# alazarteka/Self-Forcing

Hardware: AMD Instinct MI355X
Metric: decoded frames/sec/node, Wan-1.3B 832x480 4-step AR rollout (higher is better)
Workload: dtype bf16

## Files before the change

self-forcing_amd/csrc/dit_forward.hip:

```cpp
#include <algorithm>
#include "sf_host.h"

int sf_internal_write_kv_indices(void* buf, int layers, int64_t global_end, int64_t local_end, void* stream);

namespace {

struct Work {
  void *x, *xn, *qkv, *q, *att, *hbuf, *cols, *headout, *sin, *etmp, *e, *e0, *ctx1, *ctx;
  void* xq;
  float* xs;
  size_t total;
};

constexpr int FP8_MAX_SEGMENTS = 8;

Work carve(const sf_model* m, void* ws, int B, int F, int lat_h, int lat_w, int groups) {
  const size_t M = (size_t)B * F * (lat_h / 2) * (lat_w / 2);
  const size_t C = m->dim, BG = (size_t)B * groups, T = (size_t)B * m->text_len;
  Carve c(ws);
  Work w;
  w.x = c.take(M * C * 2);
  w.xn = c.take(M * C * 2);
  w.qkv = c.take(M * 3 * C * 2);
  w.q = c.take(M * C * 2);
  w.att = c.take(M * C * 2);
  w.hbuf = c.take(M * (size_t)m->ffn_dim * 2);
  w.cols = c.take(M * (size_t)m->in_dim * 4 * 2);
  w.headout = c.take(M * (size_t)m->out_dim * 4 * 2);
  w.sin = c.take(BG * m->freq_dim * 2);
  w.etmp = c.take(BG * C * 2);
  w.e = c.take(BG * C * 2);
  w.e0 = c.take(BG * 6 * C * 2);
  w.ctx1 = c.take(T * C * 2);
// ... 157 lines not shown
    const int T = B * m->text_len;
    SF_TRY(lin(Gemm(a->prompt_embeds, m->text_dim, m->text0_w, m->text_dim, ws.ctx1, C, T, C, m->text_dim).bias(m->text0_b).epi(SF_EPI_BIAS_GELU)
                   .fp8w(m->text0_q, m->text0_s, T)));
    SF_TRY(lin(Gemm(ws.ctx1, C, m->text2_w, C, ws.ctx, C, T, C, C).bias(m->text2_b).fp8w(m->text2_q, m->text2_s, T)));
    if (f8) SF_TRY(sf_quantize_fp8(ws.ctx, C, T, C, T, ws.xq, ws.xs, stream));
    for (int l = 0; l < m->num_layers; ++l) {
      const sf_layer_weights& lw = m->layers_host[l];
      const sf_layer_fp8& lq = f8 ? m->layers_fp8_host[l] : no_fp8;
      SF_TRY(run(Gemm(ws.ctx, C, lw.ckv_w, C, a->ck_cache_host[l], C, T, C, C).bias(lw.ckv_b).fp8w(lq.ckv_q, lq.ckv_s, T)));
      SF_TRY(sf_rmsnorm(a->ck_cache_host[l], C, lw.cnorm_k_w, a->ck_cache_host[l], C, T, C, m->eps, stream));
      SF_TRY(run(Gemm(ws.ctx, C, bptr(lw.ckv_w, (size_t)C * C), C, a->cv_cache_host[l], C, T, C, C).bias(bptr(lw.ckv_b, C))
                     .fp8w(f8 ? (const char*)lq.ckv_q + (size_t)C * C : nullptr, f8 ? lq.ckv_s + C : nullptr, T)));
    }
    if (cross_keys) SF_TRY(sf_cross_fold_scan(a->ck_cache_host, a->cv_cache_host, m->num_layers, B, m->text_len, C, cross_keys, cross_log2w, stream));
    if (im) {
      const ImgWork iw = carve_img(m, im, a->workspace, ws.total, B);
      const int R = B * im->clip_len, D = im->clip_dim;
      void* ctx_raw = iw.ctx;
      void* ctx_img = (void*)bptr(iw.ctx, (size_t)R * C);
      SF_TRY(sf_layernorm_rows(ia->clip_feature, im->img_ln0_w, im->img_ln0_b, iw.t0, R, D, im->img_eps, stream));
      SF_TRY(Gemm(iw.t0, D, im->img_fc1_w, D, iw.t1, D, R, D, D).bias(im->img_fc1_b).bf16(stream));
      SF_TRY(sf_clip_gelu(iw.t1, iw.t1, (int64_t)R * D, stream));
      SF_TRY(Gemm(iw.t1, D, im->img_fc2_w, D, ctx_raw, C, R, C, D).bias(im->img_fc2_b).bf16(stream));
      SF_TRY(sf_layernorm_affine(ctx_raw, im->img_ln1_w, im->img_ln1_b, ctx_img, R, C, im->img_eps, stream));
      for (int l = 0; l < m->num_layers; ++l) {
        const sf_i2v_layer& il = im->layers_host[l];
        SF_TRY(Gemm(ctx_img, C, il.kvimg_w, C, ia->kimg_cache_host[l], C, R, C, C).bias(il.kvimg_b).bf16(stream));
        SF_TRY(sf_rmsnorm(ia->kimg_cache_host[l], C, il.norm_k_img_w, ia->kimg_cache_host[l], C, R, C, m->eps, stream));
        SF_TRY(Gemm(ctx_img, C, bptr(il.kvimg_w, (size_t)C * C), C, ia->vimg_cache_host[l], C, R, C, C).bias(bptr(il.kvimg_b, C)).bf16(stream));
      }
    }
  }

  for (int l = 0; l < m->num_layers; ++l) {
    const sf_layer_weights& lw = m->layers_host[l];
    const sf_layer_fp8& lq = f8 ? m->layers_fp8_host[l] : no_fp8;
    const void* mod = lw.modulation;
    const bool last_layer = l == m->num_layers - 1;
    SF_TRY(sf_layernorm_modulate(ws.x, ws.xn, Mt, C, m->eps, bptr(mod, 0), bptr(mod, C), bptr(ws.e0, 0), bptr(ws.e0, C), 6L * C, rpg, stream));
    SF_TRY(lin(Gemm(ws.xn, C, lw.qkv_w, C, ws.qkv, 3 * C, Mt, 3 * C, C).bias(lw.qkv_b).fp8w(lq.qkv_q, lq.qkv_s, M)));
    for (int p = 0; p < np; ++p) {
      const sf_forward_args* q = ps[p];
      const size_t roff = (size_t)p * M;
      if (q->evict > 0) {
        SF_TRY(sf_kv_evict(q->k_cache_host[l], B, q->cache_tokens, C, q->sink_tokens, q->evict, q->keep, q->evict_scratch, q->evict_scratch_bytes, stream));
        SF_TRY(sf_kv_evict(q->v_cache_host[l], B, q->cache_tokens, C, q->sink_tokens, q->evict, q->keep, q->evict_scratch, q->evict_scratch_bytes, stream));
      }
      SF_TRY(sf_qkv_norm_rope_cache(bptr(ws.qkv, roff * 3 * C), lw.norm_q_w, lw.norm_k_w, (void*)bptr(ws.q, roff * C), q->k_cache_host[l], q->v_cache_host[l],
                                    m->rope_cos, m->rope_sin, B, F, h, w, C, m->num_heads, q->cache_tokens, q->write_start, q->start_frame, m->eps, stream));
      if (q->cache_only && last_layer) continue;
      SF_TRY(Attention(bptr(ws.q, roff * C), C, (long)L * C, bptr(q->k_cache_host[l], (size_t)q->attn_start * C), bptr(q->v_cache_host[l], (size_t)q->attn_start * C),
                       C, cache_b, (void*)bptr(ws.att, roff * C), C, (long)L * C, B, m->num_heads, L, q->attn_end - q->attn_start).run(stream));
    }
    const int p0 = last_layer ? first_full : 0;
    if (p0 == np) return finish_indices();
    const size_t r0 = (size_t)p0 * M;
    const int Mr = (np - p0) * M;
    void* x = (void*)bptr(ws.x, r0 * C);
    void* xn = (void*)bptr(ws.xn, r0 * C);
    void* qb = (void*)bptr(ws.q, r0 * C);
    void* att = (void*)bptr(ws.att, r0 * C);
    void* hb = (void*)bptr(ws.hbuf, r0 * m->ffn_dim);
    const void* e0r = bptr(ws.e0, (size_t)p0 * BG * 6 * C);
    SF_TRY(lin(Gemm(att, C, lw.o_w, C, x, C, Mr, C, C).bias(lw.o_b).epi(SF_EPI_BIAS_GATE_RESID).resid(x, C)
                   .gate(bptr(mod, 2 * (size_t)C), bptr(e0r, 2 * (size_t)C), 6L * C, rpg).fp8w(lq.o_q, lq.o_s, M)));
    SF_TRY(sf_layernorm_affine(x, lw.norm3_w, lw.norm3_b, xn, Mr, C, m->eps, stream));
    SF_TRY(lin(Gemm(xn, C, lw.cq_w, C, qb, C, Mr, C, C).bias(lw.cq_b).fp8w(lq.cq_q, lq.cq_s, M)));
    SF_TRY(sf_rmsnorm(qb, C, lw.cnorm_q_w, qb, C, Mr, C, m->eps, stream));
    for (int p = p0; p < np; ++p)
      SF_TRY(Attention(bptr(ws.q, (size_t)p * M * C), C, (long)L * C, a->ck_cache_host[l], a->cv_cache_host[l], C, ctx_b, (void*)bptr(ws.att, (size_t)p * M * C), C,
                       (long)L * C, B, m->num_heads, L, m->text_len)
                 .fold(cross_keys ? cross_keys + (size_t)l * B : nullptr, cross_keys ? cross_log2w + (size_t)l * B : nullptr).run(stream));
    if (im)
      SF_TRY(Attention(ws.q, C, (long)L * C, ia->kimg_cache_host[l], ia->vimg_cache_host[l], C, (long)im->clip_len * C, ws.att, C, (long)L * C, B, m->num_heads, L,
                       im->clip_len).accum().run(stream));
    SF_TRY(lin(Gemm(att, C, lw.co_w, C, x, C, Mr, C, C).bias(lw.co_b).epi(SF_EPI_BIAS_RESID).resid(x, C).fp8w(lq.co_q, lq.co_s, M)));
    SF_TRY(sf_layernorm_modulate(x, xn, Mr, C, m->eps, bptr(mod, 3 * (size_t)C), bptr(mod, 4 * (size_t)C), bptr(e0r, 3 * (size_t)C),
                                 bptr(e0r, 4 * (size_t)C), 6L * C, rpg, stream));
    SF_TRY(lin(Gemm(xn, C, lw.ffn0_w, C, hb, m->ffn_dim, Mr, m->ffn_dim, C).bias(lw.ffn0_b).epi(SF_EPI_BIAS_GELU).fp8w(lq.ffn0_q, lq.ffn0_s, M)));
    SF_TRY(lin(Gemm(hb, m->ffn_dim, lw.ffn2_w, m->ffn_dim, x, C, Mr, C, m->ffn_dim).bias(lw.ffn2_b).epi(SF_EPI_BIAS_GATE_RESID).resid(x, C)
                   .gate(bptr(mod, 5 * (size_t)C), bptr(e0r, 5 * (size_t)C), 6L * C, rpg).fp8w(lq.ffn2_q, lq.ffn2_s, M)));
  }
// ... 15 lines not shown
```

self-forcing_amd/csrc/elementwise.hip:

```cpp
#include "sf_common.h"
#include "../../include/sf_hip.h"

namespace {

constexpr int ROWS_PER_BLOCK = 4;

template <int NCH>
__device__ __forceinline__ void load_row(const bf16_t* row, int lane, float (&v)[NCH][8]) {
#pragma unroll
  for (int i = 0; i < NCH; ++i) {
    const bf16x8 t = *reinterpret_cast<const bf16x8*>(row + (i * 64 + lane) * 8);
#pragma unroll
    for (int j = 0; j < 8; ++j) v[i][j] = (float)t[j];
  }
}

template <int NCH>
__device__ __forceinline__ void ln_stats(const float (&v)[NCH][8], int C, float eps, float& mean, float& rstd) {
  float s = 0.f;
#pragma unroll
  for (int i = 0; i < NCH; ++i)
#pragma unroll
    for (int j = 0; j < 8; ++j) s += v[i][j];
  mean = wave_sum(s) / (float)C;
// ... 70 lines not shown
#pragma unroll
      for (int j = 0; j < 8; ++j)
        o[j] = (bf16_t)((v[i][j] - mean) * rstd * (MODE == 0 ? 1.0f + (float)scl[i][j] : (float)scl[i][j]) + (float)add[i][j]);
      *reinterpret_cast<bf16x8*>(out + (long)row * C + (i * 64 + lane) * 8) = o;
    }
  }
}

template <int NCH>
__global__ __launch_bounds__(256) void rmsnorm_kernel(const bf16_t* __restrict__ x, int ldx, const bf16_t* __restrict__ w,
                                                      bf16_t* __restrict__ out, int ldo, int M, int C, float eps) {
  const int lane = threadIdx.x & 63;
  const int row = blockIdx.x * ROWS_PER_BLOCK + (threadIdx.x >> 6);
  if (row >= M) return;
  float v[NCH][8];
  load_row<NCH>(x + (long)row * ldx, lane, v);
  float q = 0.f;
#pragma unroll
  for (int i = 0; i < NCH; ++i)
#pragma unroll
    for (int j = 0; j < 8; ++j) q += v[i][j] * v[i][j];
  const float r = rsqrtf(wave_sum(q) / (float)C + eps);
#pragma unroll
  for (int i = 0; i < NCH; ++i) {
    const int e = (i * 64 + lane) * 8;
    const bf16x8 wt = *reinterpret_cast<const bf16x8*>(w + e);
    bf16x8 o;
#pragma unroll
    for (int j = 0; j < 8; ++j) o[j] = (bf16_t)((float)(bf16_t)(v[i][j] * r) * (float)wt[j]);
    *reinterpret_cast<bf16x8*>(out + (long)row * ldo + e) = o;
  }
}

template <int NCH>
__global__ __launch_bounds__(256) void qkv_norm_rope_cache_kernel(
    const bf16_t* __restrict__ qkv, const bf16_t* __restrict__ wq, const bf16_t* __restrict__ wk,
    bf16_t* __restrict__ q_out, bf16_t* __restrict__ k_cache, bf16_t* __restrict__ v_cache,
    const float* __restrict__ rope_cos, const float* __restrict__ rope_sin, int rows, int L, int hgt, int wid, int C,
    long cache_tokens, int write_start, int start_frame, float eps, int c0, int c1) {
  const int lane = threadIdx.x & 63;
  const int row = blockIdx.x * ROWS_PER_BLOCK + (threadIdx.x >> 6);
  if (row >= rows) return;
  const int b = row / L, t = row - b * L;
  const int fi = t / (hgt * wid), rem = t - fi * (hgt * wid);
  const int hi = rem / wid, wi = rem - hi * wid;
  const int pos_t = start_frame + fi;
  const bf16_t* src = qkv + (long)row * 3 * C;
  const long crow = ((long)b * cache_tokens + write_start + t) * C;

#pragma unroll
  for (int i = 0; i < NCH; ++i) {
    const int e = (i * 64 + lane) * 8;
    *reinterpret_cast<u32x4*>(v_cache + crow + e) = *reinterpret_cast<const u32x4*>(src + 2 * C + e);
  }

#pragma unroll
  for (int which = 0; which < 2; ++which) {
    float v[NCH][8];
    load_row<NCH>(src + which * C, lane, v);
    float q = 0.f;
#pragma unroll
    for (int i = 0; i < NCH; ++i)
#pragma unroll
      for (int j = 0; j < 8; ++j) q += v[i][j] * v[i][j];
    const float r = rsqrtf(wave_sum(q) / (float)C + eps);
    const bf16_t* wn = which ? wk : wq;
    bf16_t* dst = which ? (k_cache + crow) : (q_out + (long)row * C);
#pragma unroll
    for (int i = 0; i < NCH; ++i) {
      const int e = (i * 64 + lane) * 8;
      const bf16x8 wt = *reinterpret_cast<const bf16x8*>(wn + e);
      const int pair0 = (e & 127) >> 1;
      bf16x8 o;
#pragma unroll
      for (int pp = 0; pp < 4; ++pp) {
        const int pj = pair0 + pp;
        const int pos = pj < c0 ? pos_t : (pj < c0 + c1 ? hi : wi);
        const float cs = rope_cos[pos * 64 + pj];
        const float sn = rope_sin[pos * 64 + pj];
        const float re = (float)(bf16_t)((float)(bf16_t)(v[i][2 * pp] * r) * (float)wt[2 * pp]);
        const float im = (float)(bf16_t)((float)(bf16_t)(v[i][2 * pp + 1] * r) * (float)wt[2 * pp + 1]);
        o[2 * pp] = (bf16_t)(re * cs - im * sn);
        o[2 * pp + 1] = (bf16_t)(re * sn + im * cs);
      }
      *reinterpret_cast<bf16x8*>(dst + e) = o;
    }
  }
}

__global__ __launch_bounds__(256) void copy_rows_kernel(const char* __restrict__ src, long src_bstride,
                                                        char* __restrict__ dst, long dst_bstride, long bytes_per_batch) {
  const long n16 = bytes_per_batch >> 4;
  const char* s = src + (long)blockIdx.y * src_bstride;
  char* d = dst + (long)blockIdx.y * dst_bstride;
  for (long i = (long)blockIdx.x * blockDim.x + threadIdx.x; i < n16; i += (long)gridDim.x * blockDim.x)
    reinterpret_cast<u32x4*>(d)[i] = reinterpret_cast<const u32x4*>(s)[i];
}

__global__ __launch_bounds__(256) void patchify_kernel(const bf16_t* __restrict__ x, bf16_t* __restrict__ cols, long total,
                                                       int Cin, int H, int W) {
  const int h2 = H >> 1, w2 = W >> 1;
  for (long i = (long)blockIdx.x * blockDim.x + threadIdx.x; i < total; i += (long)gridDim.x * blockDim.x) {
    const int cch = (int)(i % Cin);
    long r = i / Cin;
    const int ww = (int)(r % w2); r /= w2;
    const int hh = (int)(r % h2);
    const long bf = r / h2;
    const bf16_t* s = x + ((bf * Cin + cch) * H + 2 * hh) * (long)W + 2 * ww;
    bf16x4 o;
    o[0] = s[0]; o[1] = s[1]; o[2] = s[W]; o[3] = s[W + 1];
    *reinterpret_cast<bf16x4*>(cols + ((bf * h2 + hh) * w2 + ww) * (long)(Cin * 4) + cch * 4) = o;
  }
}

__device__ __forceinline__ double block_sigma_lookup(double t, const float* __restrict__ sigmas,
                                                     const float* __restrict__ timesteps, int n_table) {
// ... 144 lines not shown
                                     const void* mod_scale, const void* e0_shift, const void* e0_scale,
                                     int64_t e0_group_stride, int rows_per_group, void* stream) {
  SF_CHECK(x && out && mod_shift && mod_scale && e0_shift && e0_scale, "sf_layernorm_modulate: null tensor");
  SF_CHECK(M > 0 && channels_ok(C), "sf_layernorm_modulate: unsupported shape M=%d C=%d (C must be 512*{1,2,3,4,5,6,8,10})", M, C);
  SF_CHECK(rows_per_group > 0 && e0_group_stride % 8 == 0, "sf_layernorm_modulate: bad group layout");
  return launch_layernorm<0>((const bf16_t*)x, (bf16_t*)out, M, C, eps, (const bf16_t*)mod_shift, (const bf16_t*)mod_scale,
                             (const bf16_t*)e0_shift, (const bf16_t*)e0_scale, e0_group_stride, rows_per_group,
                             "sf_layernorm_modulate", (hipStream_t)stream);
}

extern "C" int sf_layernorm_affine(const void* x, const void* weight, const void* bias, void* out, int M, int C,
                                   float eps, void* stream) {
  SF_CHECK(x && out && weight && bias, "sf_layernorm_affine: null tensor");
  SF_CHECK(M > 0 && channels_ok(C), "sf_layernorm_affine: unsupported shape M=%d C=%d", M, C);
  return launch_layernorm<1>((const bf16_t*)x, (bf16_t*)out, M, C, eps, (const bf16_t*)weight, (const bf16_t*)bias, nullptr,
                             nullptr, 0, 1, "sf_layernorm_affine", (hipStream_t)stream);
}

extern "C" int sf_rmsnorm(const void* x, int ldx, const void* weight, void* out, int ldo, int M, int C, float eps,
                          void* stream) {
  SF_CHECK(x && out && weight, "sf_rmsnorm: null tensor");
  SF_CHECK(M > 0 && channels_ok(C) && ldx >= C && ldo >= C && ldx % 8 == 0 && ldo % 8 == 0, "sf_rmsnorm: unsupported shape M=%d C=%d", M, C);
  const dim3 grid((M + ROWS_PER_BLOCK - 1) / ROWS_PER_BLOCK), block(256);
  hipStream_t s = (hipStream_t)stream;
  switch (C / 512) {
#define SF_RMS_CASE(N) \
  case N: return sf_launch<&rmsnorm_kernel<N>>("sf_rmsnorm", grid, block, 0, s, (const bf16_t*)x, ldx, (const bf16_t*)weight, (bf16_t*)out, ldo, M, C, eps);
    SF_RMS_CASE(1) SF_RMS_CASE(2) SF_RMS_CASE(3) SF_RMS_CASE(4) SF_RMS_CASE(5) SF_RMS_CASE(6) SF_RMS_CASE(8) SF_RMS_CASE(10)
#undef SF_RMS_CASE
    default: SF_CHECK(false, "sf_rmsnorm: unsupported channel count %d", C);
  }
}

extern "C" int sf_qkv_norm_rope_cache(const void* qkv, const void* norm_q_w, const void* norm_k_w, void* q_out,
                                      void* k_cache, void* v_cache, const float* rope_cos, const float* rope_sin,
                                      int B, int f, int h, int w, int C, int num_heads, int64_t cache_tokens,
                                      int write_start, int start_frame, float eps, void* stream) {
  SF_CHECK(qkv && norm_q_w && norm_k_w && q_out && k_cache && v_cache && rope_cos && rope_sin, "sf_qkv_norm_rope_cache: null tensor");
  SF_CHECK(B > 0 && f > 0 && h > 0 && w > 0 && channels_ok(C), "sf_qkv_norm_rope_cache: unsupported shape");
  SF_CHECK(num_heads > 0 && C == num_heads * 128, "sf_qkv_norm_rope_cache: head_dim must be 128 (C=%d heads=%d)", C, num_heads);
  const int L = f * h * w;
  SF_CHECK(write_start >= 0 && (int64_t)write_start + L <= cache_tokens, "sf_qkv_norm_rope_cache: cache overflow: write_start=%d + L=%d > capacity=%lld",
           write_start, L, (long long)cache_tokens);
  SF_CHECK(start_frame >= 0 && start_frame + f <= 1024 && h <= 1024 && w <= 1024, "sf_qkv_norm_rope_cache: RoPE position out of the 1024-entry table");
  const int rows = B * L;
  const dim3 grid((rows + ROWS_PER_BLOCK - 1) / ROWS_PER_BLOCK), block(256);
  hipStream_t s = (hipStream_t)stream;
  const int c = 64, c1 = c / 3, c0 = c - 2 * c1;
  switch (C / 512) {
#define SF_QKV_CASE(N)                                                                                                                         \
  case N: return sf_launch<&qkv_norm_rope_cache_kernel<N>>("sf_qkv_norm_rope_cache", grid, block, 0, s, (const bf16_t*)qkv, (const bf16_t*)norm_q_w, \
                             (const bf16_t*)norm_k_w, (bf16_t*)q_out, (bf16_t*)k_cache, (bf16_t*)v_cache, rope_cos, rope_sin,                    \
                             rows, L, h, w, C, (long)cache_tokens, write_start, start_frame, eps, c0, c1);
    SF_QKV_CASE(1) SF_QKV_CASE(2) SF_QKV_CASE(3) SF_QKV_CASE(4) SF_QKV_CASE(5) SF_QKV_CASE(6) SF_QKV_CASE(8) SF_QKV_CASE(10)
#undef SF_QKV_CASE
    default: SF_CHECK(false, "sf_qkv_norm_rope_cache: unsupported channel count %d", C);
  }
}

extern "C" int sf_kv_evict(void* cache, int B, int64_t cache_tokens, int row_elems, int sink, int evict, int keep,
                           void* scratch, size_t scratch_bytes, void* stream) {
  SF_CHECK(cache && B > 0 && row_elems > 0 && (row_elems % 8) == 0, "sf_kv_evict: bad arguments");
  SF_CHECK(sink >= 0 && evict >= 0 && keep >= 0 && (int64_t)sink + evict + keep <= cache_tokens, "sf_kv_evict: window out of range");
  if (evict == 0 || keep == 0) return 0;
  const long row_b = (long)row_elems * 2;
  const long bytes = (long)keep * row_b;
  SF_CHECK(scratch && scratch_bytes >= (size_t)(bytes * B), "sf_kv_evict: scratch too small (%zu < %ld)", scratch_bytes, bytes * B);
  char* base = (char*)cache;
  const long bstride = (long)cache_tokens * row_b;
  const int gx = (int)min((long)2048, (bytes / 16 + 255) / 256);
  const dim3 grid(gx, B), block(256);
  hipStream_t s = (hipStream_t)stream;
  SF_TRY(sf_launch<&copy_rows_kernel>("sf_kv_evict", grid, block, 0, s, base + (long)(sink + evict) * row_b, bstride, (char*)scratch, bytes, bytes));
  return sf_launch<&copy_rows_kernel>("sf_kv_evict", grid, block, 0, s, (const char*)scratch, bytes, base + (long)sink * row_b, bstride, bytes);
}

extern "C" int sf_patchify(const void* x, void* cols, int B, int F, int Cin, int H, int W, void* stream) {
  SF_CHECK(x && cols && B > 0 && F > 0 && Cin > 0, "sf_patchify: bad arguments");
  SF_CHECK(H % 2 == 0 && W % 2 == 0, "sf_patchify: latent H=%d W=%d must be even (patch 2x2)", H, W);
  const long total = (long)B * F * (H / 2) * (W / 2) * Cin;
  const int gx = (int)min((long)4096, (total + 255) / 256);
  return sf_launch<&patchify_kernel>("sf_patchify", dim3(gx), dim3(256), 0, (hipStream_t)stream, (const bf16_t*)x, (bf16_t*)cols, total, Cin, H, W);
}

extern "C" int sf_unpatchify_x0(const void* head_out, const void* xt, const void* timestep, int t_is_int64,
                                const float* sigmas, const float* timesteps, int n_table, void* flow, void* x0,
                                int B, int F, int groups, int Cout, int H, int W, void* stream) {
  SF_CHECK(head_out && xt && timestep && sigmas && timesteps && flow && x0, "sf_unpatchify_x0: null tensor");
  SF_CHECK(B > 0 && F > 0 && groups > 0 && F % groups == 0, "sf_unpatchify_x0: frames=%d not divisible by groups=%d", F, groups);
  SF_CHECK(H % 2 == 0 && W % 2 == 0 && n_table > 0, "sf_unpatchify_x0: bad shape");
// ... 104 lines not shown
```

self-forcing_amd/csrc/gemm_bf16.hip:

```cpp
#include <type_traits>
#include "sf_common.h"
#include "lds_dma.h"
#include "../../include/sf_hip.h"

namespace {

constexpr int BM = 128, BN = 128, BK = 64;
constexpr int GEMM_THREADS = 256;
constexpr int TILE_BYTES = BM * BK * 2;
constexpr int STAGE_BYTES = 2 * TILE_BYTES;
constexpr int GEMM_LDS = 2 * STAGE_BYTES;

struct GemmP {
  const bf16_t* a;
  const bf16_t* w;
  const bf16_t* bias;
  bf16_t* out;
  const bf16_t* resid;
  const bf16_t* gate_mod;
  const bf16_t* gate_e0;
  long gate_group_stride;
  int rows_per_group;
  int M, N, K, lda, ldw, ldo, ldr;
  int tiles_m, tiles_n;
  long a_bs, w_bs, o_bs, r_bs;
  const float* a_scale;
  const float* w_scale;
  int rows_per_seg;
};

typedef int i32x4 __attribute__((ext_vector_type(4)));
typedef int i32x8 __attribute__((ext_vector_type(8)));

__device__ __forceinline__ f32x4 mfma_f8(const bf16x8& w0, const bf16x8& w1, const bf16x8& x0, const bf16x8& x1, const f32x4& acc) {
  const i32x8 wv = __builtin_shufflevector(__builtin_bit_cast(i32x4, w0), __builtin_bit_cast(i32x4, w1), 0, 1, 2, 3, 4, 5, 6, 7);
  const i32x8 xv = __builtin_shufflevector(__builtin_bit_cast(i32x4, x0), __builtin_bit_cast(i32x4, x1), 0, 1, 2, 3, 4, 5, 6, 7);
  return __builtin_amdgcn_mfma_scale_f32_16x16x128_f8f6f4(wv, xv, acc, 0, 0, 0, 127, 0, 127);
}

template <int MT>
__device__ __forceinline__ void fp8_scale_acc(const GemmP& p, f32x4 (&acc)[MT][4], int m_base, int n_base, int lane) {
  f32x4 ws[4];
#pragma unroll
  for (int nt = 0; nt < 4; ++nt) ws[nt] = *reinterpret_cast<const f32x4*>(p.w_scale + min(n_base + nt * 16 + (lane >> 4) * 4, p.N - 4));
#pragma unroll
  for (int mt = 0; mt < MT; ++mt) {
    const float sa = p.a_scale[min(m_base + mt * 16 + (lane & 15), p.M - 1) / p.rows_per_seg];
#pragma unroll
    for (int nt = 0; nt < 4; ++nt)
#pragma unroll
      for (int j = 0; j < 4; ++j) acc[mt][nt][j] = acc[mt][nt][j] * (sa * ws[nt][j]);
  }
}

template <int EPI>
__device__ __forceinline__ bf16x4 epi_apply(const GemmP& p, const f32x4& a4, int m, int n, const bf16_t* e0row) {
  float y[4];
#pragma unroll
  for (int j = 0; j < 4; ++j) y[j] = a4[j];
  if (p.bias) {
    const bf16x4 b = *reinterpret_cast<const bf16x4*>(p.bias + n);
#pragma unroll
    for (int j = 0; j < 4; ++j) y[j] += (float)b[j];
  }
  if (EPI == SF_EPI_BIAS_GELU) {
#pragma unroll
    for (int j = 0; j < 4; ++j) y[j] = gelu_tanh_f(y[j]);
  }
  if (EPI == SF_EPI_BIAS_GATE_RESID) {
    const bf16x4 gm = *reinterpret_cast<const bf16x4*>(p.gate_mod + n);
    const bf16x4 ge = *reinterpret_cast<const bf16x4*>(e0row + n);
#pragma unroll
    for (int j = 0; j < 4; ++j) y[j] *= (float)(bf16_t)((float)gm[j] + (float)ge[j]);
  }
  if (EPI == SF_EPI_BIAS_RESID || EPI == SF_EPI_BIAS_GATE_RESID) {
    const bf16x4 rv = *reinterpret_cast<const bf16x4*>(p.resid + (long)m * p.ldr + n);
#pragma unroll
    for (int j = 0; j < 4; ++j) y[j] += (float)rv[j];
  }
  bf16x4 o;
#pragma unroll
  for (int j = 0; j < 4; ++j) o[j] = (bf16_t)y[j];
  return o;
}

template <int EPI, int MT>
__device__ __forceinline__ void gemm_epilogue(const GemmP& p, f32x4 (&acc)[MT][4], int mrow, int ncol) {
#pragma unroll
  for (int mt = 0; mt < MT; ++mt) {
    const int m = mrow + mt * 16;
    if (m >= p.M) continue;
    const bf16_t* e0row = nullptr;
    if (EPI == SF_EPI_BIAS_GATE_RESID) e0row = p.gate_e0 + (long)(m / p.rows_per_group) * p.gate_group_stride;
#pragma unroll
    for (int nt = 0; nt < 4; ++nt) {
      const int n = ncol + nt * 16;
      if (n >= p.N) continue;
      if (EPI == SF_EPI_F32) {
        *reinterpret_cast<f32x4*>(reinterpret_cast<float*>(p.out) + (long)m * p.ldo + n) = acc[mt][nt];
        continue;
      }
      *reinterpret_cast<bf16x4*>(p.out + (long)m * p.ldo + n) = epi_apply<EPI>(p, acc[mt][nt], m, n, e0row);
    }
  }
}

template <int EPI>
__device__ __forceinline__ bf16x4 epi_math(const f32x4& a4, const bf16x4& b, const bf16x4& gm, const bf16x4& ge, const bf16x4& rv) {
  float y[4];
#pragma unroll
  for (int j = 0; j < 4; ++j) y[j] = a4[j] + (float)b[j];
  if (EPI == SF_EPI_BIAS_GELU) {
#pragma unroll
    for (int j = 0; j < 4; ++j) y[j] = gelu_tanh_f(y[j]);
  }
  if (EPI == SF_EPI_BIAS_GATE_RESID) {
#pragma unroll
    for (int j = 0; j < 4; ++j) y[j] *= (float)(bf16_t)((float)gm[j] + (float)ge[j]);
  }
  if (EPI == SF_EPI_BIAS_RESID || EPI == SF_EPI_BIAS_GATE_RESID) {
#pragma unroll
    for (int j = 0; j < 4; ++j) y[j] += (float)rv[j];
  }
  bf16x4 o;
#pragma unroll
  for (int j = 0; j < 4; ++j) o[j] = (bf16_t)y[j];
  return o;
}

template <int EPI, int MT>
__device__ __forceinline__ void gemm_epilogue_lds(const GemmP& p, f32x4 (&acc)[MT][4], int m_base, int n_base, char* wbuf, int lane) {
  const int r16 = lane & 15, cg = lane >> 4;
  constexpr bool GATE = EPI == SF_EPI_BIAS_GATE_RESID;
  constexpr bool RESID = EPI == SF_EPI_BIAS_RESID || EPI == SF_EPI_BIAS_GATE_RESID;
  const bf16x4 zero4 = {(bf16_t)0.f, (bf16_t)0.f, (bf16_t)0.f, (bf16_t)0.f};
// ... 13 lines not shown
#pragma unroll
    for (int nt = 0; nt < 4; ++nt) gm_v[nt] = *reinterpret_cast<const bf16x4*>(p.gate_mod + ncol[nt]);
  }
  constexpr int MB = 4;
#pragma unroll
  for (int m0 = 0; m0 < MT; m0 += MB) {
    bf16x4 rv[MB][4], ge[MB][4];
#pragma unroll
    for (int i = 0; i < MB; ++i) {
      if (m0 + i >= MT) break;
      const int m = min(m_base + (m0 + i) * 16 + r16, p.M - 1);
      const bf16_t* e0row = GATE ? p.gate_e0 + (long)(m / p.rows_per_group) * p.gate_group_stride : nullptr;
#pragma unroll
      for (int nt = 0; nt < 4; ++nt) {
        rv[i][nt] = RESID ? *reinterpret_cast<const bf16x4*>(p.resid + (long)m * p.ldr + ncol[nt]) : zero4;
        ge[i][nt] = GATE ? *reinterpret_cast<const bf16x4*>(e0row + ncol[nt]) : zero4;
      }
    }
#pragma unroll
    for (int i = 0; i < MB; ++i) {
      if (m0 + i >= MT) break;
      const int row = (m0 + i) * 16 + r16;
#pragma unroll
      for (int nt = 0; nt < 4; ++nt) {
        const int col = nt * 16 + cg * 4;
        const bf16x4 o = epi_math<EPI>(acc[m0 + i][nt], bias_v[nt], gm_v[nt], ge[i][nt], rv[i][nt]);
        const int chunk = (col >> 3) ^ (row & 7);
        *reinterpret_cast<bf16x4*>(wbuf + row * 128 + (chunk << 4) + (col & 4) * 2) = o;
      }
    }
  }
  __builtin_amdgcn_s_waitcnt(0xc07f);
  const int rr = lane >> 3, ch = lane & 7;
#pragma unroll
  for (int i = 0; i < 2 * MT; ++i) {
    const int row = i * 8 + rr;
    const int m = m_base + row, n = n_base + ch * 8;
    const bf16x8 v = *reinterpret_cast<const bf16x8*>(wbuf + row * 128 + ((ch ^ (row & 7)) << 4));
    if (m < p.M && n < p.N) *reinterpret_cast<bf16x8*>(p.out + (long)m * p.ldo + n) = v;
  }
}

template <int EPI, bool F8>
__global__ __launch_bounds__(GEMM_THREADS, 2) void gemm_bf16_kernel(GemmP p) {
  extern __shared__ __attribute__((aligned(16))) char smem[];
  const int tid = threadIdx.x;
  const int lane = tid & 63;
  const int wave = __builtin_amdgcn_readfirstlane(tid >> 6);

  if (blockIdx.y) {
    const long bz = blockIdx.y;
    p.a += bz * p.a_bs; p.w += bz * p.w_bs;
    if (EPI == SF_EPI_F32) p.out = reinterpret_cast<bf16_t*>(reinterpret_cast<float*>(p.out) + bz * p.o_bs); else p.out += bz * p.o_bs;
    if (p.resid) p.resid += bz * p.r_bs;
  }
  const int nwg = gridDim.x, bid = blockIdx.x;
  const int wg = sf_xcd_remap(bid, nwg);
  constexpr int GROUP_M = 8;
  const int width = GROUP_M * p.tiles_n;
  const int group = wg / width, first_m = group * GROUP_M;
  const int gsz = min(p.tiles_m - first_m, GROUP_M);
  const int in_group = wg - group * width;
  const int tm = first_m + in_group % gsz, tn = in_group / gsz;
  const int m0 = tm * BM, n0 = tn * BN;

  const bf16_t* a_src[4];
// ... 494 lines not shown
    return st == SF_GEMM_PP256 ? launch_pp_epi<8, F8>(p, a->epilogue, name, s)
         : st == SF_GEMM_PP224 ? launch_pp_epi<7, F8>(p, a->epilogue, name, s)
         : st == SF_GEMM_PP192 ? launch_pp_epi<6, F8>(p, a->epilogue, name, s) : launch_pp2_epi<F8>(p, a->epilogue, name, s);
  const int batch = a->batch > 1 ? a->batch : 1;
  p.a_bs = a->a_bstride; p.w_bs = a->w_bstride; p.o_bs = a->o_bstride; p.r_bs = a->r_bstride;
  SF_CHECK(batch == 1 || (a->a_bstride % 8 == 0 && a->w_bstride % 8 == 0 && a->o_bstride % 4 == 0 && a->r_bstride % 4 == 0),
           "%s: batch strides must keep 16-byte (operands) / 8-byte (output) alignment", name);
  const dim3 grid(p.tiles_m * p.tiles_n, batch), block(GEMM_THREADS);
  switch (a->epilogue) {
    case SF_EPI_BIAS: return sf_launch<&gemm_bf16_kernel<SF_EPI_BIAS, F8>>(name, grid, block, GEMM_LDS, s, p);
    case SF_EPI_BIAS_GELU: return sf_launch<&gemm_bf16_kernel<SF_EPI_BIAS_GELU, F8>>(name, grid, block, GEMM_LDS, s, p);
    case SF_EPI_BIAS_RESID: return sf_launch<&gemm_bf16_kernel<SF_EPI_BIAS_RESID, F8>>(name, grid, block, GEMM_LDS, s, p);
    case SF_EPI_BIAS_GATE_RESID: return sf_launch<&gemm_bf16_kernel<SF_EPI_BIAS_GATE_RESID, F8>>(name, grid, block, GEMM_LDS, s, p);
    case SF_EPI_F32:
      if constexpr (F8) {
        SF_CHECK(false, "%s: the raw fp32 epilogue is bf16-only", name);
      } else {
        SF_CHECK((uintptr_t)a->out % 16 == 0, "%s: fp32 output must be 16-byte aligned", name);
        return sf_launch<&gemm_bf16_kernel<SF_EPI_F32, false>>(name, grid, block, GEMM_LDS, s, p);
      }
    default: SF_CHECK(false, "%s: unknown epilogue %d", name, a->epilogue);
  }
}

void fill_params(const sf_gemm_args* a, GemmP& p, int unit) {
  p.a = (const bf16_t*)a->a; p.w = (const bf16_t*)a->w; p.bias = (const bf16_t*)a->bias;
  p.out = (bf16_t*)a->out; p.resid = (const bf16_t*)a->resid;
  p.gate_mod = (const bf16_t*)a->gate_mod; p.gate_e0 = (const bf16_t*)a->gate_e0;
  p.gate_group_stride = a->gate_group_stride; p.rows_per_group = a->rows_per_group;
  p.M = a->M; p.N = a->N; p.K = a->K / unit; p.lda = a->lda / unit; p.ldw = a->ldw / unit; p.ldo = a->ldo; p.ldr = a->ldr;
  p.tiles_n = (a->N + BN - 1) / BN;
  p.tiles_m = (a->M + BM - 1) / BM;
  p.a_scale = nullptr; p.w_scale = nullptr; p.rows_per_seg = 1;
}

}

extern "C" int sf_gemm_bf16(const sf_gemm_args* a, void* stream) {
  if (const int rc = check_args(a, "sf_gemm_bf16", BK)) return rc;
  GemmP p;
  fill_params(a, p, 1);
  return run_gemm<false>(a, p, "sf_gemm_bf16", (hipStream_t)stream);
}

extern "C" int sf_gemm_fp8(const sf_gemm_args* a, const float* a_scale, int rows_per_segment, const float* w_scale, void* stream) {
  if (const int rc = check_args(a, "sf_gemm_fp8", 2 * BK)) return rc;
  SF_CHECK(a->batch <= 1, "sf_gemm_fp8: batched products are bf16-only");
  SF_CHECK(a_scale && w_scale && rows_per_segment > 0, "sf_gemm_fp8: needs a_scale, w_scale and rows_per_segment > 0");
  SF_CHECK((uintptr_t)w_scale % 16 == 0, "sf_gemm_fp8: w_scale must be 16-byte aligned");
  GemmP p;
  fill_params(a, p, 2);
  p.a_scale = a_scale; p.w_scale = w_scale; p.rows_per_seg = rows_per_segment;
  return run_gemm<true>(a, p, "sf_gemm_fp8", (hipStream_t)stream);
}
```

self-forcing_amd/csrc/sf_host.h:

```cpp
#pragma once
#include <cstring>
#include "sf_common.h"
#include "../../include/sf_hip.h"

inline int sf_hip_ok(hipError_t e, const char* who, const char* what) {
  SF_CHECK(e == hipSuccess, "%s: %s failed: %s", who, what, hipGetErrorString(e));
  return 0;
}

struct Carve {
  char* base;
  size_t off;
  explicit Carve(void* p) : base((char*)p), off(0) {}
  char* take(size_t bytes) {
    char* r = base ? base + off : nullptr;
    off += (bytes + 255) & ~(size_t)255;
    return r;
  }
};

struct Gemm {
  sf_gemm_args g;
  const void* wq = nullptr;
  const float* w_scale = nullptr;
  int rows_per_segment = 0;
  Gemm(const void* a, int lda, const void* w, int ldw, void* out, int ldo, int M, int N, int K) {
    memset(&g, 0, sizeof(g));
    g.a = a; g.lda = lda; g.w = w; g.ldw = ldw; g.out = out; g.ldo = ldo; g.M = M; g.N = N; g.K = K;
    g.epilogue = SF_EPI_BIAS;
    g.rows_per_group = 1;
  }
  Gemm& bias(const void* b) { g.bias = b; return *this; }
  Gemm& epi(int e) { g.epilogue = e; return *this; }
  Gemm& resid(const void* r, int ldr) { g.resid = r; g.ldr = ldr; return *this; }
  Gemm& gate(const void* gate_mod, const void* gate_e0, long group_stride, int rows_per_group) {
    g.gate_mod = gate_mod; g.gate_e0 = gate_e0; g.gate_group_stride = group_stride; g.rows_per_group = rows_per_group;
    return *this;
  }
  Gemm& batch(int n, long a_bstride, long w_bstride, long o_bstride) {
    g.batch = n; g.a_bstride = a_bstride; g.w_bstride = w_bstride; g.o_bstride = o_bstride;
    return *this;
  }
  Gemm& fp8w(const void* w_e4m3, const float* scale, int rows_per_seg) {
    wq = w_e4m3; w_scale = scale; rows_per_segment = rows_per_seg;
    return *this;
  }
  int bf16(void* stream) const { return sf_gemm_bf16(&g, stream); }
  int fp8(const void* aq, const float* a_scale, void* stream) const {
    sf_gemm_args q = g;
    q.a = aq; q.lda = g.K; q.w = wq;
    return sf_gemm_fp8(&q, a_scale, rows_per_segment, w_scale, stream);
  }
};

struct Attention {
  sf_attention_args a;
  Attention(const void* q, long q_stride, long q_bstride, const void* k, const void* v, long kv_stride, long kv_bstride, void* out,
            long o_stride, long o_bstride, int B, int H, int Lq, int Lk) {
    memset(&a, 0, sizeof(a));
    a.q = q; a.q_stride = q_stride; a.q_bstride = q_bstride;
    a.k = k; a.v = v; a.kv_stride = kv_stride; a.kv_bstride = kv_bstride;
    a.out = out; a.o_stride = o_stride; a.o_bstride = o_bstride;
    a.B = B; a.H = H; a.Lq = Lq; a.Lk = Lk;
    a.structure = SF_ATTN_AUTO;
  }
  Attention& structure(int s) { a.structure = s; return *this; }
  Attention& accum() { a.accumulate = 1; return *this; }
  Attention& fold(const int32_t* keys, const float* log2w) { a.keys = keys; a.log2w = log2w; return *this; }
  int run(void* stream) const { return sf_attention(&a, stream); }
};
```

Baseline: 95.73.

## Write V columns of QKV GEMM directly into the KV cache

Adds a split-store epilogue to the bf16/fp8 GEMM so output columns past 2*C (the V projection) go straight into the per-layer V cache at each pass's write_start. The separate V copy in the qkv norm/rope kernel is then skipped. The kernel also preloads Q/K rows and rope tables up front. This removes one read and write of the V slice per layer. It is on by default but falls back when eviction is active or the two passes' cache regions overlap, and it adds per-row address math in the GEMM epilogue.

```diff
diff --git a/self-forcing_amd/csrc/dit_forward.hip b/self-forcing_amd/csrc/dit_forward.hip
--- a/self-forcing_amd/csrc/dit_forward.hip
+++ b/self-forcing_amd/csrc/dit_forward.hip
@@ -1,4 +1,5 @@
 #include <algorithm>
+#include <cstdlib>
 #include "sf_host.h"
 
 int sf_internal_write_kv_indices(void* buf, int layers, int64_t global_end, int64_t local_end, void* stream);
@@ -222,13 +223,32 @@
     }
   }
 
+  bool v_direct = true;
+  if (const char* e = getenv("SF_V_DIRECT")) v_direct = !(e[0] == '0' && e[1] == 0);
+  for (int p = 0; p < np; ++p) v_direct = v_direct && ps[p]->evict <= 0;
+  if (np == 2) {
+    const sf_forward_args *p0 = ps[0], *p1 = ps[1];
+    const int w1 = p1->write_start;
+    v_direct = v_direct && (w1 + L <= p0->attn_start || w1 >= p0->attn_end) && (w1 + L <= p0->write_start || w1 >= p0->write_start + L);
+  }
+  int qkv_structure = SF_GEMM_AUTO;
+  if (const char* e = getenv("SF_V_DIRECT_GEMM")) qkv_structure = atoi(e);
+
   for (int l = 0; l < m->num_layers; ++l) {
     const sf_layer_weights& lw = m->layers_host[l];
     const sf_layer_fp8& lq = f8 ? m->layers_fp8_host[l] : no_fp8;
     const void* mod = lw.modulation;
     const bool last_layer = l == m->num_layers - 1;
     SF_TRY(sf_layernorm_modulate(ws.x, ws.xn, Mt, C, m->eps, bptr(mod, 0), bptr(mod, C), bptr(ws.e0, 0), bptr(ws.e0, C), 6L * C, rpg, stream));
-    SF_TRY(lin(Gemm(ws.xn, C, lw.qkv_w, C, ws.qkv, 3 * C, Mt, 3 * C, C).bias(lw.qkv_b).fp8w(lq.qkv_q, lq.qkv_s, M)));
+    sf_gemm_split vsplit = {};
+    if (v_direct) {
+      vsplit.dst = a->v_cache_host[l];
+      vsplit.split_n = 2 * C; vsplit.ld = C;
+      vsplit.rows_per_sample = L; vsplit.samples = B; vsplit.passes = np;
+      vsplit.sample_rows = (long)a->cache_tokens; vsplit.sample_stride = cache_b;
+      for (int p = 0; p < np; ++p) vsplit.first_row[p] = ps[p]->write_start;
+    }
+    SF_TRY(lin(Gemm(ws.xn, C, lw.qkv_w, C, ws.qkv, 3 * C, Mt, 3 * C, C).bias(lw.qkv_b).fp8w(lq.qkv_q, lq.qkv_s, M).structure(qkv_structure).split(vsplit)));
     for (int p = 0; p < np; ++p) {
       const sf_forward_args* q = ps[p];
       const size_t roff = (size_t)p * M;
@@ -236,8 +256,12 @@
         SF_TRY(sf_kv_evict(q->k_cache_host[l], B, q->cache_tokens, C, q->sink_tokens, q->evict, q->keep, q->evict_scratch, q->evict_scratch_bytes, stream));
         SF_TRY(sf_kv_evict(q->v_cache_host[l], B, q->cache_tokens, C, q->sink_tokens, q->evict, q->keep, q->evict_scratch, q->evict_scratch_bytes, stream));
       }
-      SF_TRY(sf_qkv_norm_rope_cache(bptr(ws.qkv, roff * 3 * C), lw.norm_q_w, lw.norm_k_w, (void*)bptr(ws.q, roff * C), q->k_cache_host[l], q->v_cache_host[l],
-                                    m->rope_cos, m->rope_sin, B, F, h, w, C, m->num_heads, q->cache_tokens, q->write_start, q->start_frame, m->eps, stream));
+      if (v_direct)
+        SF_TRY(sf_internal_qk_norm_rope_cache(bptr(ws.qkv, roff * 3 * C), lw.norm_q_w, lw.norm_k_w, (void*)bptr(ws.q, roff * C), q->k_cache_host[l], m->rope_cos,
+                                              m->rope_sin, B, F, h, w, C, m->num_heads, q->cache_tokens, q->write_start, q->start_frame, m->eps, stream));
+      else
+        SF_TRY(sf_qkv_norm_rope_cache(bptr(ws.qkv, roff * 3 * C), lw.norm_q_w, lw.norm_k_w, (void*)bptr(ws.q, roff * C), q->k_cache_host[l], q->v_cache_host[l],
+                                      m->rope_cos, m->rope_sin, B, F, h, w, C, m->num_heads, q->cache_tokens, q->write_start, q->start_frame, m->eps, stream));
       if (q->cache_only && last_layer) continue;
       SF_TRY(Attention(bptr(ws.q, roff * C), C, (long)L * C, bptr(q->k_cache_host[l], (size_t)q->attn_start * C), bptr(q->v_cache_host[l], (size_t)q->attn_start * C),
                        C, cache_b, (void*)bptr(ws.att, roff * C), C, (long)L * C, B, m->num_heads, L, q->attn_end - q->attn_start).run(stream));
diff --git a/self-forcing_amd/csrc/elementwise.hip b/self-forcing_amd/csrc/elementwise.hip
--- a/self-forcing_amd/csrc/elementwise.hip
+++ b/self-forcing_amd/csrc/elementwise.hip
@@ -126,7 +126,7 @@
   }
 }
 
-template <int NCH>
+template <int NCH, bool COPY_V>
 __global__ __launch_bounds__(256) void qkv_norm_rope_cache_kernel(
     const bf16_t* __restrict__ qkv, const bf16_t* __restrict__ wq, const bf16_t* __restrict__ wk,
     bf16_t* __restrict__ q_out, bf16_t* __restrict__ k_cache, bf16_t* __restrict__ v_cache,
@@ -142,16 +142,40 @@
   const bf16_t* src = qkv + (long)row * 3 * C;
   const long crow = ((long)b * cache_tokens + write_start + t) * C;
 
+  bf16x8 raw[2][NCH];
+#pragma unroll
+  for (int which = 0; which < 2; ++which)
+#pragma unroll
+    for (int i = 0; i < NCH; ++i) raw[which][i] = *reinterpret_cast<const bf16x8*>(src + which * C + (i * 64 + lane) * 8);
+  float cs[NCH][4], sn[NCH][4];
 #pragma unroll
   for (int i = 0; i < NCH; ++i) {
-    const int e = (i * 64 + lane) * 8;
-    *reinterpret_cast<u32x4*>(v_cache + crow + e) = *reinterpret_cast<const u32x4*>(src + 2 * C + e);
+    const int pair0 = (((i * 64 + lane) * 8) & 127) >> 1;
+#pragma unroll
+    for (int pp = 0; pp < 4; ++pp) {
+      const int pj = pair0 + pp;
+      const int pos = pj < c0 ? pos_t : (pj < c0 + c1 ? hi : wi);
+      cs[i][pp] = rope_cos[pos * 64 + pj];
+      sn[i][pp] = rope_sin[pos * 64 + pj];
+    }
+  }
+  if constexpr (NCH <= 4) __builtin_amdgcn_sched_barrier(0);
+
+  if constexpr (COPY_V) {
+#pragma unroll
+    for (int i = 0; i < NCH; ++i) {
+      const int e = (i * 64 + lane) * 8;
+      *reinterpret_cast<u32x4*>(v_cache + crow + e) = *reinterpret_cast<const u32x4*>(src + 2 * C + e);
+    }
   }
 
 #pragma unroll
   for (int which = 0; which < 2; ++which) {
     float v[NCH][8];
-    load_row<NCH>(src + which * C, lane, v);
+#pragma unroll
+    for (int i = 0; i < NCH; ++i)
+#pragma unroll
+      for (int j = 0; j < 8; ++j) v[i][j] = (float)raw[which][i][j];
     float q = 0.f;
 #pragma unroll
     for (int i = 0; i < NCH; ++i)
@@ -164,18 +188,13 @@
     for (int i = 0; i < NCH; ++i) {
       const int e = (i * 64 + lane) * 8;
       const bf16x8 wt = *reinterpret_cast<const bf16x8*>(wn + e);
-      const int pair0 = (e & 127) >> 1;
       bf16x8 o;
 #pragma unroll
       for (int pp = 0; pp < 4; ++pp) {
-        const int pj = pair0 + pp;
-        const int pos = pj < c0 ? pos_t : (pj < c0 + c1 ? hi : wi);
-        const float cs = rope_cos[pos * 64 + pj];
-        const float sn = rope_sin[pos * 64 + pj];
         const float re = (float)(bf16_t)((float)(bf16_t)(v[i][2 * pp] * r) * (float)wt[2 * pp]);
         const float im = (float)(bf16_t)((float)(bf16_t)(v[i][2 * pp + 1] * r) * (float)wt[2 * pp + 1]);
-        o[2 * pp] = (bf16_t)(re * cs - im * sn);
-        o[2 * pp + 1] = (bf16_t)(re * sn + im * cs);
+        o[2 * pp] = (bf16_t)(re * cs[i][pp] - im * sn[i][pp]);
+        o[2 * pp + 1] = (bf16_t)(re * sn[i][pp] + im * cs[i][pp]);
       }
       *reinterpret_cast<bf16x8*>(dst + e) = o;
     }
@@ -386,11 +405,11 @@
   }
 }
 
-extern "C" int sf_qkv_norm_rope_cache(const void* qkv, const void* norm_q_w, const void* norm_k_w, void* q_out,
-                                      void* k_cache, void* v_cache, const float* rope_cos, const float* rope_sin,
-                                      int B, int f, int h, int w, int C, int num_heads, int64_t cache_tokens,
-                                      int write_start, int start_frame, float eps, void* stream) {
-  SF_CHECK(qkv && norm_q_w && norm_k_w && q_out && k_cache && v_cache && rope_cos && rope_sin, "sf_qkv_norm_rope_cache: null tensor");
+namespace {
+int launch_qkv_norm_rope_cache(const void* qkv, const void* norm_q_w, const void* norm_k_w, void* q_out, void* k_cache, void* v_cache,
+                               const float* rope_cos, const float* rope_sin, int B, int f, int h, int w, int C, int num_heads,
+                               int64_t cache_tokens, int write_start, int start_frame, float eps, void* stream) {
+  SF_CHECK(qkv && norm_q_w && norm_k_w && q_out && k_cache && rope_cos && rope_sin, "sf_qkv_norm_rope_cache: null tensor");
   SF_CHECK(B > 0 && f > 0 && h > 0 && w > 0 && channels_ok(C), "sf_qkv_norm_rope_cache: unsupported shape");
   SF_CHECK(num_heads > 0 && C == num_heads * 128, "sf_qkv_norm_rope_cache: head_dim must be 128 (C=%d heads=%d)", C, num_heads);
   const int L = f * h * w;
@@ -401,15 +420,36 @@
   const dim3 grid((rows + ROWS_PER_BLOCK - 1) / ROWS_PER_BLOCK), block(256);
   hipStream_t s = (hipStream_t)stream;
   const int c = 64, c1 = c / 3, c0 = c - 2 * c1;
+#define SF_QKV_LAUNCH(N, V)                                                                                                                       \
+  sf_launch<&qkv_norm_rope_cache_kernel<N, V>>("sf_qkv_norm_rope_cache", grid, block, 0, s, (const bf16_t*)qkv, (const bf16_t*)norm_q_w,         \
+                                               (const bf16_t*)norm_k_w, (bf16_t*)q_out, (bf16_t*)k_cache, (bf16_t*)v_cache, rope_cos, rope_sin, \
+                                               rows, L, h, w, C, (long)cache_tokens, write_start, start_frame, eps, c0, c1)
+#define SF_QKV_CASE(N) \
+  case N: return v_cache ? SF_QKV_LAUNCH(N, true) : SF_QKV_LAUNCH(N, false);
   switch (C / 512) {
-#define SF_QKV_CASE(N)                                                                                                                         \
-  case N: return sf_launch<&qkv_norm_rope_cache_kernel<N>>("sf_qkv_norm_rope_cache", grid, block, 0, s, (const bf16_t*)qkv, (const bf16_t*)norm_q_w, \
-                             (const bf16_t*)norm_k_w, (bf16_t*)q_out, (bf16_t*)k_cache, (bf16_t*)v_cache, rope_cos, rope_sin,                    \
-                             rows, L, h, w, C, (long)cache_tokens, write_start, start_frame, eps, c0, c1);
     SF_QKV_CASE(1) SF_QKV_CASE(2) SF_QKV_CASE(3) SF_QKV_CASE(4) SF_QKV_CASE(5) SF_QKV_CASE(6) SF_QKV_CASE(8) SF_QKV_CASE(10)
+    default: SF_CHECK(false, "sf_qkv_norm_rope_cache: unsupported channel count %d", C);
+  }
 #undef SF_QKV_CASE
-    default: SF_CHECK(false, "sf_qkv_norm_rope_cache: unsupported channel count %d", C);
-  }
+#undef SF_QKV_LAUNCH
+}
+}
+
+extern "C" int sf_qkv_norm_rope_cache(const void* qkv, const void* norm_q_w, const void* norm_k_w, void* q_out,
+                                      void* k_cache, void* v_cache, const float* rope_cos, const float* rope_sin,
+                                      int B, int f, int h, int w, int C, int num_heads, int64_t cache_tokens,
+                                      int write_start, int start_frame, float eps, void* stream) {
+  SF_CHECK(v_cache, "sf_qkv_norm_rope_cache: null tensor");
+  return launch_qkv_norm_rope_cache(qkv, norm_q_w, norm_k_w, q_out, k_cache, v_cache, rope_cos, rope_sin, B, f, h, w, C, num_heads, cache_tokens,
+                                    write_start, start_frame, eps, stream);
+}
+
+__attribute__((visibility("hidden"))) int sf_internal_qk_norm_rope_cache(const void* qkv, const void* norm_q_w, const void* norm_k_w, void* q_out,
+                                                                         void* k_cache, const float* rope_cos, const float* rope_sin, int B, int f,
+                                                                         int h, int w, int C, int num_heads, int64_t cache_tokens, int write_start,
+                                                                         int start_frame, float eps, void* stream) {
+  return launch_qkv_norm_rope_cache(qkv, norm_q_w, norm_k_w, q_out, k_cache, nullptr, rope_cos, rope_sin, B, f, h, w, C, num_heads, cache_tokens,
+                                    write_start, start_frame, eps, stream);
 }
 
 extern "C" int sf_kv_evict(void* cache, int B, int64_t cache_tokens, int row_elems, int sink, int evict, int keep,
diff --git a/self-forcing_amd/csrc/gemm_bf16.hip b/self-forcing_amd/csrc/gemm_bf16.hip
--- a/self-forcing_amd/csrc/gemm_bf16.hip
+++ b/self-forcing_amd/csrc/gemm_bf16.hip
@@ -1,7 +1,6 @@
 #include <type_traits>
-#include "sf_common.h"
+#include "sf_host.h"
 #include "lds_dma.h"
-#include "../../include/sf_hip.h"
 
 namespace {
 
@@ -27,7 +26,15 @@
   const float* a_scale;
   const float* w_scale;
   int rows_per_seg;
+  bf16_t* out2;
+  long sample_stride2;
+  int split_n, ld2, rows2, samples2, first_row2_0, first_row2_1;
 };
+
+__device__ __forceinline__ bf16_t* split_row(const GemmP& p, int s, int r) {
+  const int pass = s >= p.samples2;
+  return p.out2 + (long)(s - pass * p.samples2) * p.sample_stride2 + (long)((pass ? p.first_row2_1 : p.first_row2_0) + r) * p.ld2;
+}
 
 typedef int i32x4 __attribute__((ext_vector_type(4)));
 typedef int i32x8 __attribute__((ext_vector_type(8)));
@@ -92,6 +99,8 @@
     if (m >= p.M) continue;
     const bf16_t* e0row = nullptr;
     if (EPI == SF_EPI_BIAS_GATE_RESID) e0row = p.gate_e0 + (long)(m / p.rows_per_group) * p.gate_group_stride;
+    bf16_t* row2 = nullptr;
+    if (EPI == SF_EPI_BIAS && p.out2) row2 = split_row(p, m / p.rows2, m % p.rows2);
 #pragma unroll
     for (int nt = 0; nt < 4; ++nt) {
       const int n = ncol + nt * 16;
@@ -100,7 +109,8 @@
         *reinterpret_cast<f32x4*>(reinterpret_cast<float*>(p.out) + (long)m * p.ldo + n) = acc[mt][nt];
         continue;
       }
-      *reinterpret_cast<bf16x4*>(p.out + (long)m * p.ldo + n) = epi_apply<EPI>(p, acc[mt][nt], m, n, e0row);
+      bf16_t* dst = row2 && n >= p.split_n ? row2 + (n - p.split_n) : p.out + (long)m * p.ldo + n;
+      *reinterpret_cast<bf16x4*>(dst) = epi_apply<EPI>(p, acc[mt][nt], m, n, e0row);
     }
   }
 }
@@ -180,6 +190,19 @@
   }
   __builtin_amdgcn_s_waitcnt(0xc07f);
   const int rr = lane >> 3, ch = lane & 7;
+  if (EPI == SF_EPI_BIAS && p.out2 && n_base >= p.split_n) {
+    int s = (m_base + rr) / p.rows2, r = (m_base + rr) - s * p.rows2;
+#pragma unroll
+    for (int i = 0; i < 2 * MT; ++i) {
+      const int row = i * 8 + rr;
+      const int m = m_base + row, n = n_base + ch * 8;
+      const bf16x8 v = *reinterpret_cast<const bf16x8*>(wbuf + row * 128 + ((ch ^ (row & 7)) << 4));
+      if (m < p.M && n < p.N) *reinterpret_cast<bf16x8*>(split_row(p, s, r) + (n - p.split_n)) = v;
+      r += 8;
+      while (r >= p.rows2) { r -= p.rows2; ++s; }
+    }
+    return;
+  }
 #pragma unroll
   for (int i = 0; i < 2 * MT; ++i) {
     const int row = i * 8 + rr;
@@ -740,18 +763,38 @@
   p.tiles_n = (a->N + BN - 1) / BN;
   p.tiles_m = (a->M + BM - 1) / BM;
   p.a_scale = nullptr; p.w_scale = nullptr; p.rows_per_seg = 1;
-}
-
-}
-
-extern "C" int sf_gemm_bf16(const sf_gemm_args* a, void* stream) {
+  p.out2 = nullptr; p.sample_stride2 = 0;
+  p.split_n = 0; p.ld2 = 0; p.rows2 = 1; p.samples2 = 1; p.first_row2_0 = 0; p.first_row2_1 = 0;
+}
+
+int set_split(const sf_gemm_args* a, const sf_gemm_split* sp, GemmP& p, const char* name) {
+  if (!sp) return 0;
+  SF_CHECK(sp->dst && (uintptr_t)sp->dst % 16 == 0, "%s: split store needs a 16-byte aligned destination", name);
+  SF_CHECK(a->epilogue == SF_EPI_BIAS && a->batch <= 1, "%s: split store is built for the SF_EPI_BIAS epilogue of one product", name);
+  SF_CHECK(sp->split_n > 0 && sp->split_n % 64 == 0 && sp->split_n < a->N, "%s: split_n=%d must be a multiple of 64 inside N=%d", name, sp->split_n, a->N);
+  SF_CHECK(sp->ld % 8 == 0 && sp->ld >= a->N - sp->split_n && sp->sample_stride % 8 == 0, "%s: split store needs ld %% 8 == 0, ld >= N - split_n", name);
+  SF_CHECK(sp->rows_per_sample > 0 && sp->samples > 0 && sp->passes >= 1 && sp->passes <= 2 &&
+               (long)a->M == (long)sp->passes * sp->samples * sp->rows_per_sample,
+           "%s: split store: M=%d is not passes x samples x rows_per_sample = %d x %d x %d", name, a->M, sp->passes, sp->samples, sp->rows_per_sample);
+  for (int i = 0; i < sp->passes; ++i)
+    SF_CHECK(sp->first_row[i] >= 0 && (long)sp->first_row[i] + sp->rows_per_sample <= sp->sample_rows &&
+                 (long)sp->sample_rows * sp->ld <= sp->sample_stride,
+             "%s: split store: rows [%d, %d + %d) leave a sample's %ld rows", name, sp->first_row[i], sp->first_row[i], sp->rows_per_sample, (long)sp->sample_rows);
+  p.out2 = (bf16_t*)sp->dst; p.sample_stride2 = sp->sample_stride;
+  p.split_n = sp->split_n; p.ld2 = sp->ld; p.rows2 = sp->rows_per_sample; p.samples2 = sp->samples;
+  p.first_row2_0 = sp->first_row[0]; p.first_row2_1 = sp->passes > 1 ? sp->first_row[1] : 0;
+  return 0;
+}
+
+int gemm_bf16(const sf_gemm_args* a, const sf_gemm_split* sp, void* stream) {
   if (const int rc = check_args(a, "sf_gemm_bf16", BK)) return rc;
   GemmP p;
   fill_params(a, p, 1);
+  SF_TRY(set_split(a, sp, p, "sf_gemm_bf16"));
   return run_gemm<false>(a, p, "sf_gemm_bf16", (hipStream_t)stream);
 }
 
-extern "C" int sf_gemm_fp8(const sf_gemm_args* a, const float* a_scale, int rows_per_segment, const float* w_scale, void* stream) {
+int gemm_fp8(const sf_gemm_args* a, const sf_gemm_split* sp, const float* a_scale, int rows_per_segment, const float* w_scale, void* stream) {
   if (const int rc = check_args(a, "sf_gemm_fp8", 2 * BK)) return rc;
   SF_CHECK(a->batch <= 1, "sf_gemm_fp8: batched products are bf16-only");
   SF_CHECK(a_scale && w_scale && rows_per_segment > 0, "sf_gemm_fp8: needs a_scale, w_scale and rows_per_segment > 0");
@@ -759,5 +802,20 @@
   GemmP p;
   fill_params(a, p, 2);
   p.a_scale = a_scale; p.w_scale = w_scale; p.rows_per_seg = rows_per_segment;
+  SF_TRY(set_split(a, sp, p, "sf_gemm_fp8"));
   return run_gemm<true>(a, p, "sf_gemm_fp8", (hipStream_t)stream);
 }
+
+}
+
+extern "C" int sf_gemm_bf16(const sf_gemm_args* a, void* stream) { return gemm_bf16(a, nullptr, stream); }
+
+extern "C" int sf_gemm_fp8(const sf_gemm_args* a, const float* a_scale, int rows_per_segment, const float* w_scale, void* stream) {
+  return gemm_fp8(a, nullptr, a_scale, rows_per_segment, w_scale, stream);
+}
+
+__attribute__((visibility("hidden"))) int sf_internal_gemm_split(const sf_gemm_args* a, const sf_gemm_split* sp, const float* a_scale,
+                                                                 int rows_per_segment, const float* w_scale, void* stream) {
+  SF_CHECK(sp != nullptr, "sf_internal_gemm_split: null split");
+  return a_scale ? gemm_fp8(a, sp, a_scale, rows_per_segment, w_scale, stream) : gemm_bf16(a, sp, stream);
+}
diff --git a/self-forcing_amd/csrc/sf_host.h b/self-forcing_amd/csrc/sf_host.h
--- a/self-forcing_amd/csrc/sf_host.h
+++ b/self-forcing_amd/csrc/sf_host.h
@@ -19,11 +19,25 @@
   }
 };
 
+struct sf_gemm_split {
+  void* dst;
+  int split_n, ld;
+  int rows_per_sample, samples, passes;
+  long sample_rows, sample_stride;
+  int first_row[2];
+};
+int sf_internal_gemm_split(const sf_gemm_args* a, const sf_gemm_split* sp, const float* a_scale, int rows_per_segment, const float* w_scale,
+                           void* stream);
+int sf_internal_qk_norm_rope_cache(const void* qkv, const void* norm_q_w, const void* norm_k_w, void* q_out, void* k_cache, const float* rope_cos,
+                                   const float* rope_sin, int B, int f, int h, int w, int C, int num_heads, int64_t cache_tokens, int write_start,
+                                   int start_frame, float eps, void* stream);
+
 struct Gemm {
   sf_gemm_args g;
   const void* wq = nullptr;
   const float* w_scale = nullptr;
   int rows_per_segment = 0;
+  sf_gemm_split sp2 = {};
   Gemm(const void* a, int lda, const void* w, int ldw, void* out, int ldo, int M, int N, int K) {
     memset(&g, 0, sizeof(g));
     g.a = a; g.lda = lda; g.w = w; g.ldw = ldw; g.out = out; g.ldo = ldo; g.M = M; g.N = N; g.K = K;
@@ -45,10 +59,13 @@
     wq = w_e4m3; w_scale = scale; rows_per_segment = rows_per_seg;
     return *this;
   }
-  int bf16(void* stream) const { return sf_gemm_bf16(&g, stream); }
+  Gemm& structure(int s) { g.structure = s; return *this; }
+  Gemm& split(const sf_gemm_split& sp) { sp2 = sp; return *this; }
+  int bf16(void* stream) const { return sp2.dst ? sf_internal_gemm_split(&g, &sp2, nullptr, 0, nullptr, stream) : sf_gemm_bf16(&g, stream); }
   int fp8(const void* aq, const float* a_scale, void* stream) const {
     sf_gemm_args q = g;
     q.a = aq; q.lda = g.K; q.w = wq;
+    if (sp2.dst) return sf_internal_gemm_split(&q, &sp2, a_scale, rows_per_segment, w_scale, stream);
     return sf_gemm_fp8(&q, a_scale, rows_per_segment, w_scale, stream);
   }
 };
```

After: 96.33, median of 6. Within noise of the previous version (+0.6%).
